# zhuhaozh/metadrive_ped

Hardware: AMD Instinct MI355X
Metric: agent-steps/sec at 4096 envs x 240-beam lidar (higher is better)
Workload: dtype f32; 1 GPU; BASELINE configs[1]: 4096 batched MetaDriveEnv per GPU, 3-block PG map (reference default block distribution: curves, straights, ramps, X/T intersections, roundabouts), 240-beam lidar, traffic_density=0.1, trigger traffic, auto-reset; envs_per_gpu=4096, agents_per_env=1, mover_capacity=24, n_beams=240

## Files before the change

### metadrive_ped_amd/csrc/mdstep.hip

```cpp
#include <hip/hip_runtime.h>
#include <stddef.h>
#include <stdint.h>
#include <stdio.h>
#include <stdlib.h>

#include <type_traits>

#include "md_curriculum.h"
#include "md_expert.h"
#include "md_expert_sense.h"
#include "md_ai_protect.h"
#include "md_scenario.h"
#include "md_topdown.h"
#include "md_render.h"
#include "md_branch.h"
#include "md_ped.h"
#include "md_vector_obs.h"
#include "md_lean_pins.h"
#include "md_lean_view.h"

namespace {

constexpr int kBlock = 256;

enum Phase : int {
    PH_RESET = 1,
    PH_IDM = 2,
    PH_INTEGRATE = 4,
    PH_LOCALIZE = 8,
    PH_CONTACTS = 16,
    PH_TRAFFIC = 32,
    PH_OBSERVE = 64,
    PH_LIDAR = 128,
    PH_LIFECYCLE = 256,
    PH_ALL = 511,
    PH_LOCALIZE_ROAD_FIRST = PH_LOCALIZE | (1 << 20),
};

thread_local char g_err[256] = "ok";

#ifdef MD_STAMP
__device__ unsigned long long* g_stamp_buf = nullptr;
__device__ const int* g_env_order = nullptr;
#define MD_STAMP_AT(i)                                                                         \
    do {                                                                                       \
        if (threadIdx.x == 0 && g_stamp_buf) {                                                 \
            unsigned long long* sb_ = g_stamp_buf + (size_t)blockIdx.x * 32;                   \
            sb_[(i)] = __builtin_readcyclecounter();                                           \
            if ((i) == 0) {                                                                    \
                sb_[12] = __builtin_amdgcn_s_memrealtime();                                    \
                sb_[14] = (unsigned long long)__builtin_amdgcn_s_getreg(63492) |               \
                          ((unsigned long long)__builtin_amdgcn_s_getreg(63508) << 32);        \
            }                                                                                  \
            if ((i) == 11) sb_[13] = __builtin_amdgcn_s_memrealtime();                         \
        }                                                                                      \
    } while (0)
#define MD_FINE_STAMP(cond, i)                                                                 \
    do {                                                                                       \
        if ((cond) && g_stamp_buf) g_stamp_buf[(size_t)blockIdx.x * 32 + 16 + (i)] = __builtin_readcyclecounter(); \
    } while (0)
#define MD_LOC_COUNT(cond, hit)                                                                \
    do {                                                                                       \
        if ((cond) && g_stamp_buf) {                                                           \
            atomicAdd(&g_stamp_buf[(size_t)blockIdx.x * 32 + 16 + 12], 1ull);                  \
            if (hit) atomicAdd(&g_stamp_buf[(size_t)blockIdx.x * 32 + 16 + 13], 1ull);         \
        }                                                                                      \
    } while (0)
#define MD_AHEAD_STAMP(cond, i)                                                                \
    do {                                                                                       \
        if ((cond) && g_stamp_buf) g_stamp_buf[(size_t)blockIdx.x * 32 + (i)] = __builtin_readcyclecounter(); \
    } while (0)
enum : int { MD_AHEAD_EVALUATED = 32, MD_AHEAD_HIT = 40, MD_AHEAD_MISS = 48 };
#define MD_AHEAD_COUNT(cond, what)                                                             \
    do {                                                                                       \
        if ((cond) && g_stamp_buf) atomicAdd(&g_stamp_buf[(size_t)blockIdx.x * 32 + 16 + 12], 1ull << (what)); \
    } while (0)
__device__ unsigned long long* g_contacts_buf = nullptr;
#define MD_CONTACTS_STAMP(cond, i)                                                             \
    do {                                                                                       \
        if ((cond) && g_contacts_buf) g_contacts_buf[(size_t)blockIdx.x * 8 + (i)] = __builtin_readcyclecounter(); \
    } while (0)
#define MD_CONTACTS_COUNT(cond, cells, items)                                                  \
    do {                                                                                       \
        if ((cond) && g_contacts_buf) {                                                        \
            g_contacts_buf[(size_t)blockIdx.x * 8 + 4] += (unsigned long long)(cells);         \
            g_contacts_buf[(size_t)blockIdx.x * 8 + 5] += (unsigned long long)(items);         \
        }                                                                                      \
    } while (0)
#else
#define MD_CONTACTS_STAMP(cond, i) do { } while (0)
#define MD_CONTACTS_COUNT(cond, cells, items) do { } while (0)
#define MD_STAMP_AT(i) do { } while (0)
#define MD_FINE_STAMP(cond, i) do { } while (0)
#define MD_LOC_COUNT(cond, hit) do { } while (0)
#define MD_AHEAD_STAMP(cond, i) do { } while (0)
#define MD_AHEAD_COUNT(cond, what) do { } while (0)
#endif
#ifndef MD_ENV_SKIP
#define MD_ENV_SKIP 0
#endif

__host__ __device__ constexpr uint32_t align_up(uint32_t b, uint32_t a) { return (b + a - 1) & ~(a - 1); }

__device__ __forceinline__ float bcast_f(float v, int src) { return __shfl(v, src, 64); }
__device__ __forceinline__ int bcast_i(int v, int src) { return __shfl(v, src, 64); }

__device__ __forceinline__ void wave_lds_sync() {
    __builtin_amdgcn_fence(__ATOMIC_RELEASE, "wavefront");
    __builtin_amdgcn_wave_barrier();
    __builtin_amdgcn_fence(__ATOMIC_ACQUIRE, "wavefront");
}

#ifndef MD_NT_STAGE
#define MD_NT_STAGE 1
#endif
typedef unsigned int md_u32x4 __attribute__((ext_vector_type(4)));
__device__ __forceinline__ uint4 ld_stream(const uint4* p) {
#if MD_NT_STAGE
    const md_u32x4 v = __builtin_nontemporal_load(reinterpret_cast<const md_u32x4*>(p));
    return make_uint4(v.x, v.y, v.z, v.w);
#else
    return *p;
#endif
}
__device__ __forceinline__ void st_stream(uint4* p, const uint4 v) {
#if MD_NT_STAGE
    md_u32x4 t;
    t.x = v.x; t.y = v.y; t.z = v.z; t.w = v.w;
    __builtin_nontemporal_store(t, reinterpret_cast<md_u32x4*>(p));
#else
    *p = v;
#endif
}
__device__ __forceinline__ void st_stream_f(float* p, float v) {
#if MD_NT_STAGE
    __builtin_nontemporal_store(v, p);
#else
    *p = v;
#endif
}

__device__ __forceinline__ int wave_min_i(int v, bool valid, int none) {
    unsigned long long m = __ballot(valid);
    int best = none;
    while (m) {
        const int l = __ffsll((long long)m) - 1;
        m &= m - 1;
        const int o = __shfl(v, l, 64);
        best = o < best ? o : best;
    }
    return best;
}

template <bool kLdsRow = false>
__device__ __forceinline__ void lidar_item(const MdWorld& w, const MdState& s, const MdConfig& c, int a, int sec, int lane,
                           float* __restrict__ out_row, unsigned long long* det) {
    const MdShape me = s.shape[a];
    const int beam = sec * 64 + lane;
    const bool valid = beam < c.n_beams;
    if (!md_present(me.flags)) {
        if (valid) out_row[beam] = 1.0f;
        return;
    }
    float bc = 1.0f, bs = 0.0f;
    if (valid) {
        bc = w.beam_cs[2 * beam];
        bs = w.beam_cs[2 * beam + 1];
    }
    const float dirx = (bc * me.c - bs * me.s) * c.lidar_range;
    const float diry = (bs * me.c + bc * me.s) * c.lidar_range;

    const int nb = min(64, c.n_beams - sec * 64);
    const float inv_n = __builtin_amdgcn_rcpf((float)c.n_beams);
    const float mid_rev = ((float)(sec * 64) + 0.5f * (float)(nb - 1)) * inv_n;
    const float half_rev = 0.5f * (float)(nb - 1) * inv_n;
    const float ax = __builtin_amdgcn_cosf(mid_rev), ay = __builtin_amdgcn_sinf(mid_rev);
    const float cos_h = __builtin_amdgcn_cosf(half_rev), sin_h = __builtin_amdgcn_sinf(half_rev);
    const float half_span = MD_TWO_PI_F * half_rev;
    const bool narrow = half_span < MD_HALF_PI_F - 0.02f;
    const float wax = ax * me.c - ay * me.s;
    const float way = ay * me.c + ax * me.s;

    float best = 1.0f;
    int best_j = -1;
    for (int j0 = 0; j0 < c.cap; j0 += 64) {
        const int j = j0 + lane;
        MdShape o;
        o.flags = 0;
        if (j < c.cap) o = s.shape[j];
        bool keep = (j < c.cap) && (j != a) && md_present(o.flags);
        if (keep) {
            const float ddx = o.cx - me.cx, ddy = o.cy - me.cy;
            const float d2 = ddx * ddx + ddy * ddy;
            const int k = md_kind_of(o.flags);
            const float rb = (md_is_circle_kind(k) ? o.hl : __builtin_amdgcn_sqrtf(o.hl * o.hl + o.hw * o.hw)) + 0.01f;
            const float reach = c.lidar_range + rb;
            if (d2 > reach * reach * 1.0001f) keep = false;
            else if (d2 > rb * rb) {
                const float inv = __builtin_amdgcn_rsqf(d2);
                const float sin_a = rb * inv;
                const float cos_a = __builtin_amdgcn_sqrtf(md_max(0.0f, 1.0f - sin_a * sin_a));
                if (narrow || half_span + md_asin(md_min(sin_a, 1.0f)) < MD_PI_F - 0.01f) {
                    const float cos_lim = cos_h * cos_a - sin_h * sin_a;
                    const float cos_t = (ddx * wax + ddy * way) * inv;
                    if (cos_t < cos_lim - 2e-3f) keep = false;
                }
            }
        }
        unsigned long long mask = __ballot(keep);
        while (mask) {
            const int k = __ffsll((long long)mask) - 1;
            mask &= mask - 1;
            const float ocx = bcast_f(o.cx, k), ocy = bcast_f(o.cy, k);
            const float oc = bcast_f(o.c, k), os = bcast_f(o.s, k);
            const float ohl = bcast_f(o.hl, k), ohw = bcast_f(o.hw, k);
            const int ofl = bcast_i(o.flags, k);
            const float t = md_ray_shape(me.cx, me.cy, dirx, diry, ocx, ocy, oc, os, ohl, ohw, md_kind_of(ofl));
            if (t < best) {
                best = t;
                best_j = j0 + k;
            }
        }
    }
    if (valid) {
        if (kLdsRow) out_row[beam] = best;
        else st_stream_f(&out_row[beam], best);
    }
    if (det) {
        unsigned long long todo = __ballot(valid && best_j >= 0);
        unsigned long long lo = 0ull, hi = 0ull;
        while (todo) {
            const int k = __ffsll((long long)todo) - 1;
            const int jj = bcast_i(best_j, k);
            todo &= ~__ballot(best_j == jj);
            if (jj < 64) lo |= 1ull << jj;
            else hi |= 1ull << (jj - 64);
        }
        if (lane == 0) {
            if (lo) atomicOr(&det[0], lo);
            if (hi) atomicOr(&det[1], hi);
        }
    }
}

__device__ __forceinline__ void phase_lidar(const MdWorld& w, const MdState& s, const MdConfig& c, int e, int tid, int kWaves,
// ... 340 lines not shown
        else row[out_offset1 + (i - n_beams)] = __int_as_float(l_best[k]);
    }
}

}

#include "parts/localize.inc"
#include "parts/contacts.inc"
#include "parts/idm.inc"
#include "parts/observe.inc"
#include "parts/trigger.inc"
#include "parts/lifecycle.inc"
#include "parts/lean_view.inc"

namespace {

__device__ __forceinline__ void copy16(void* dst, const void* src, int nbytes, int tid, int nthreads) {
    uint4* d = reinterpret_cast<uint4*>(dst);
    const uint4* s = reinterpret_cast<const uint4*>(src);
    for (int i = tid; i < (nbytes >> 4); i += nthreads) d[i] = s[i];
}

constexpr int kStageMaxLanes = 64;
constexpr int kWideMaxEnvs = 640;
constexpr uint32_t kRemovedMark = 0xFFFFFFFFu;

__device__ __forceinline__ int kth_bit(unsigned long long lo, unsigned long long hi, int k) {
    int slot = -1;
    while (k >= 0) {
        if (lo) {
            slot = __ffsll((long long)lo) - 1;
            lo &= lo - 1;
        } else if (hi) {
            slot = 64 + __ffsll((long long)hi) - 1;
            hi &= hi - 1;
        } else {
            return -1;
        }
        --k;
    }
    return slot;
}

struct EnvImage {
    MdShape* shape;
    MdDyn* dyn;
    MdPid* pid;
    MdParam* param;
    MdNav* nav;
    float* action;
    uint32_t* flags;
    int32_t* final_lane;
};

__device__ __forceinline__ MdState local_view(const MdState& gv, const EnvImage& img) {
    MdState s = gv;
    s.shape = img.shape;
    s.dyn = img.dyn;
    s.nav = img.nav;
    s.pid = img.pid;
    s.action = img.action;
    s.flags = img.flags;
    s.param = img.param;
    s.final_lane = img.final_lane;
    return s;
}

struct SlotMask { unsigned long long lo, hi; };
static_assert(MD_MAX_CAP <= 128, "drive_mask: two 64-bit words per env");
__device__ __forceinline__ SlotMask drive_mask(const MdShape* shape, int cap, int lane) {
    SlotMask m = {0ull, 0ull};
    for (int j0 = 0; j0 < cap; j0 += 64) {
        const int j = j0 + lane;
        const unsigned long long mk = __ballot(j < cap && md_drives(shape[j < cap ? j : 0].flags));
        if (j0 == 0) m.lo = mk;
        else m.hi = mk;
    }
    return m;
}
__device__ __forceinline__ SlotMask agent_share(SlotMask m, int agents) {
    m.lo &= agents >= 64 ? ~0ull : ((1ull << agents) - 1ull);
    m.hi &= agents <= 64 ? 0ull : (agents >= 128 ? ~0ull : ((1ull << (agents - 64)) - 1ull));
    return m;
}
__device__ __forceinline__ int popc(SlotMask m) { return __popcll(m.lo) + __popcll(m.hi); }

#ifndef MD_ENV_BLOCK
#define MD_ENV_BLOCK 256
#endif
#ifndef MD_ENV_WAVES_EU
#define MD_ENV_WAVES_EU 7
#endif
__device__ __forceinline__ void lean_pins_fold(MdState& s, MdConfig& c) {
#define MD_PIN_ZERO(f) c.f = 0;
#define MD_PIN_NUL(p) s.p = nullptr;
    MD_LEAN_PINS(MD_PIN_ZERO, MD_PIN_NUL)
#undef MD_PIN_ZERO
#undef MD_PIN_NUL
}
__device__ __forceinline__ void lean_size_pins_fold(MdConfig& c, MdConfig& c_scan) {
#define MD_PIN_EQUALS(f, v) c.f = (v);
#define MD_PIN_AT_MOST(f, v)
    MD_LEAN_SIZE_PINS(MD_PIN_EQUALS, MD_PIN_AT_MOST)
#undef MD_PIN_EQUALS
#undef MD_PIN_AT_MOST
    c_scan = c;
#define MD_PIN_EQUALS(f, v)
#define MD_PIN_AT_MOST(f, v) c_scan.f = min(c.f, (v));
    MD_LEAN_SIZE_PINS(MD_PIN_EQUALS, MD_PIN_AT_MOST)
#undef MD_PIN_EQUALS
#undef MD_PIN_AT_MOST
}

template <int PH, bool RESPAWN, bool MULTI>
constexpr int env_waves_per_eu() { return (PH == PH_ALL && !RESPAWN && !MULTI && MD_ENV_BLOCK >= 128) ? MD_ENV_WAVES_EU : 0; }

struct EnvLds { uint32_t shape, dyn, nav, pid, action, flags, lanes, roads, scratch, param, final_lane, det, onlane, cfl, tk, bytes; };
__host__ __device__ inline EnvLds env_lds(int cap, int agents, int n_lanes, int n_roads, int waves, bool multi, bool lidar_only) {
    EnvLds L;
    L.shape = 0;
    L.dyn = L.shape + (uint32_t)cap * sizeof(MdShape);
    L.nav = L.dyn + (uint32_t)cap * sizeof(MdDyn);
    L.pid = L.nav + (uint32_t)cap * sizeof(MdNav);
    L.action = L.pid + (uint32_t)cap * sizeof(MdPid);
    L.flags = L.action + (uint32_t)cap * 2 * sizeof(float);
    L.lanes = align_up(L.flags + (uint32_t)cap * sizeof(uint32_t), 16);
    L.roads = L.lanes + (uint32_t)n_lanes * sizeof(MdLane);
    L.scratch = L.roads + (uint32_t)n_roads * sizeof(MdRoad);
    L.param = L.scratch + (uint32_t)waves * (multi ? kObsScratch : 48) * sizeof(float);
    L.final_lane = L.param + (uint32_t)cap * sizeof(MdParam);
    L.det = L.final_lane + align_up(cap, 2) * sizeof(int32_t);
    L.onlane = L.det + (uint32_t)agents * 2 * sizeof(unsigned long long);
    L.cfl = L.onlane + (uint32_t)cap * sizeof(uint32_t);
    const uint32_t shared_words = 2 * cap > 8 ? 2 * cap : 8;
    L.tk = L.onlane + shared_words * sizeof(uint32_t);
    L.bytes = lidar_only ? L.dyn : L.tk + 3 * sizeof(int);
    return L;
}

template <int PH, bool STAGE_MAP, bool RESPAWN = false, bool MULTI = false, int BLK = MD_ENV_BLOCK, bool NARROW = false>
__global__ __launch_bounds__(BLK)
__attribute__((amdgpu_waves_per_eu(env_waves_per_eu<PH, RESPAWN, MULTI>() ? env_waves_per_eu<PH, RESPAWN, MULTI>() : 1,
                                   env_waves_per_eu<PH, RESPAWN, MULTI>() ? env_waves_per_eu<PH, RESPAWN, MULTI>() : 8)))
void env_kernel(MdWorld w, MdState g, MdConfig c, float* lidar_out,
                                                  int lidar_stride, int lidar_offset) {
    constexpr int kBlock = BLK;
    constexpr int kWaves = kBlock / 64;
    constexpr bool kIdmKeys = !STAGE_MAP && !RESPAWN && !MULTI;
    constexpr bool kLocRoadFirst = PH == PH_ALL ? kIdmKeys : PH == PH_LOCALIZE_ROAD_FIRST;
    constexpr bool kObsLockstep = MD_OBS_LOCKSTEP && PH == PH_ALL && kIdmKeys;
    constexpr bool kObsAhead = MD_OBS_AHEAD && kObsLockstep && kWaves > 1;
    constexpr bool kContactsFlat = MD_CONTACTS_FLAT && PH == PH_ALL && kIdmKeys;
    constexpr bool kLeanView = MD_LEAN_VIEW && PH == PH_ALL && kIdmKeys && BLK >= 256;
    LeanStageIn lean_in;
    if constexpr (kLeanView) {
        lean_in = lean_stage_in_args(lean_args_entry());
        w = MdWorld{};
        g = MdState{};
        c = MdConfig{};
        c.n_envs = lean_in.n_envs;
        c.cap = lean_in.cap;
        c.agents_per_env = lean_in.agents;
    }
    if constexpr (PH == PH_ALL && !RESPAWN && !MULTI && !STAGE_MAP) lean_pins_fold(g, c);
    static_assert(!NARROW || (PH == PH_ALL && !RESPAWN && !MULTI && !STAGE_MAP), "NARROW: a form of the lean non-staged kernel only");
    MdConfig c_scan = c;
    if constexpr (NARROW) lean_size_pins_fold(c, c_scan);
    if ((int)blockIdx.x >= c.n_envs) return;
#ifdef MD_STAMP
    const int e = g_env_order ? g_env_order[blockIdx.x] : (int)blockIdx.x;
#else
    const int e = blockIdx.x;
#endif
    const int tid = threadIdx.x;
    const int wave = tid >> 6, lane = tid & 63;
    const int cap = c.cap;

    const int n_stage_lanes = STAGE_MAP ? w.max_lanes : 0, n_stage_roads = STAGE_MAP ? w.max_roads : 0;
    constexpr bool kLidarOnly = (PH == PH_LIDAR);
    const EnvLds L = env_lds(cap, c.agents_per_env, n_stage_lanes, n_stage_roads, kWaves, MULTI, kLidarOnly);
    extern __shared__ __attribute__((aligned(16))) unsigned char smem[];
    MdShape* l_shape = reinterpret_cast<MdShape*>(smem + L.shape);
    MdDyn* l_dyn = reinterpret_cast<MdDyn*>(smem + L.dyn);
    MdNav* l_nav = reinterpret_cast<MdNav*>(smem + L.nav);
    MdPid* l_pid = reinterpret_cast<MdPid*>(smem + L.pid);
    float* l_action = reinterpret_cast<float*>(smem + L.action);
    uint32_t* l_flags = reinterpret_cast<uint32_t*>(smem + L.flags);
    MdLane* l_lanes = reinterpret_cast<MdLane*>(smem + L.lanes);
    MdRoad* l_roads = reinterpret_cast<MdRoad*>(smem + L.roads);
    float* l_scratch = reinterpret_cast<float*>(smem + L.scratch) + wave * (MULTI ? kObsScratch : 48);
    MdParam* l_param = reinterpret_cast<MdParam*>(smem + L.param);
    int32_t* l_final = reinterpret_cast<int32_t*>(smem + L.final_lane);
    unsigned long long* l_det = reinterpret_cast<unsigned long long*>(smem + L.det);
    const EnvImage img = {l_shape, l_dyn, l_pid, l_param, l_nav, l_action, l_flags, l_final};
    uint32_t* l_onlane = reinterpret_cast<uint32_t*>(smem + L.onlane);
    uint32_t* l_cfl = reinterpret_cast<uint32_t*>(smem + L.cfl);
    int* l_tk = reinterpret_cast<int*>(smem + L.tk);
    const bool track_det = (PH == PH_ALL) && (RESPAWN || MULTI) && g.detected != nullptr;

    MdState gv = md_env_view(&g, &c, e);
    const MdLane* lanes;
    const MdRoad* roads;
    if constexpr (kLeanView) lean_view_stage_in(gv, lean_in, e, cap, c.agents_per_env);
    const int reset_flag = (PH & PH_RESET) ? gv.need_reset[0] : 0;

    MD_STAMP_AT(0);
    const bool kFusedAct = (PH == PH_ALL) && gv.agent_action != nullptr;
    if (STAGE_MAP) {
        lanes = l_lanes;
        roads = l_roads;
    } else if constexpr (!kLeanView) {
        lanes = w.lanes + w.lane_off[w.env_map[e]];
        roads = w.roads + w.road_off[w.env_map[e]];
    }
    if (kLidarOnly) {
        copy16(l_shape, gv.shape, cap * (int)sizeof(MdShape), tid, kBlock);
    } else if (kBlock >= 256) {
        const int n32 = cap * 2, n64 = cap * 4;
        const uint4* g_shape = reinterpret_cast<const uint4*>(gv.shape);
        const uint4* g_dyn = reinterpret_cast<const uint4*>(gv.dyn);
        const uint4* g_pid = reinterpret_cast<const uint4*>(gv.pid);
        const uint4* g_param = reinterpret_cast<const uint4*>(gv.param);
        const uint4* g_nav = reinterpret_cast<const uint4*>(gv.nav);
        uint4 r_shape, r_dyn, r_pid, r_param, r_nav0;
        float2 r_act;
        uint32_t r_fl;
        int r_fin;
        const bool p32 = tid < n32, pc = tid < cap;
        if (p32) {
            r_shape = ld_stream(&g_shape[tid]);
            r_dyn = ld_stream(&g_dyn[tid]);
            r_pid = ld_stream(&g_pid[tid]);
            r_param = ld_stream(&g_param[tid]);
        }
        if (tid < n64) r_nav0 = ld_stream(&g_nav[tid]);
        if (pc) {
            r_act = (kFusedAct && tid < c.agents_per_env) ? reinterpret_cast<const float2*>(gv.agent_action)[tid]
                                                          : reinterpret_cast<const float2*>(gv.action)[tid];
            r_fl = gv.flags[tid];
            r_fin = gv.final_lane ? gv.final_lane[tid] : 0;
        }
        if constexpr (kLeanView) {
            lean_view_map(&lanes, &roads, lean_args_entry(), e);
            const LeanArgs kb = lean_args_here();
            const int n_envs = c.n_envs, agents = c.agents_per_env;
            lean_arg_copy(w, kb, offsetof(MdStepArgs, w));
            lean_arg_copy(c, kb, offsetof(MdStepArgs, c));
            c.n_envs = n_envs;
            c.cap = cap;
            c.agents_per_env = agents;
            lean_pins_fold(g, c);
            c_scan = c;
            if constexpr (NARROW) lean_size_pins_fold(c, c_scan);
            lean_view_routes(gv, kb, e, cap);
        }
        if (STAGE_MAP) {
            const int m = w.env_map[e];
            const int lo = w.lane_off[m], ro = w.road_off[m];
            copy16(l_lanes, w.lanes + lo, (w.lane_off[m + 1] - lo) * (int)sizeof(MdLane), tid, kBlock);
            copy16(l_roads, w.roads + ro, (w.road_off[m + 1] - ro) * (int)sizeof(MdRoad), tid, kBlock);
        }
        int tid_st = tid;
        if constexpr (kLeanView) asm("" : "+v"(tid_st));
        if (tid_st < n32) {
            reinterpret_cast<uint4*>(l_shape)[tid] = r_shape;
            reinterpret_cast<uint4*>(l_dyn)[tid] = r_dyn;
            reinterpret_cast<uint4*>(l_pid)[tid] = r_pid;
            reinterpret_cast<uint4*>(l_param)[tid] = r_param;
        }
        if (tid_st < n64) reinterpret_cast<uint4*>(l_nav)[tid] = r_nav0;
        for (int i = tid + kBlock; i < n64; i += kBlock) reinterpret_cast<uint4*>(l_nav)[i] = g_nav[i];
        if (tid_st < cap) {
            reinterpret_cast<float2*>(l_action)[tid] = r_act;
            l_flags[tid] = r_fl;
            l_final[tid] = r_fin;
        }
        if (track_det)
            for (int j = tid; j < 2 * c.agents_per_env; j += kBlock) l_det[j] = 0ull;
    } else {
        copy16(l_shape, gv.shape, cap * (int)sizeof(MdShape), tid, kBlock);
        if (STAGE_MAP) {
            const int m = w.env_map[e];
            const int lo = w.lane_off[m], ro = w.road_off[m];
            copy16(l_lanes, w.lanes + lo, (w.lane_off[m + 1] - lo) * (int)sizeof(MdLane), tid, kBlock);
            copy16(l_roads, w.roads + ro, (w.road_off[m + 1] - ro) * (int)sizeof(MdRoad), tid, kBlock);
        }
        copy16(l_dyn, gv.dyn, cap * (int)sizeof(MdDyn), tid, kBlock);
        copy16(l_nav, gv.nav, cap * (int)sizeof(MdNav), tid, kBlock);
        copy16(l_pid, gv.pid, cap * (int)sizeof(MdPid), tid, kBlock);
        copy16(l_param, gv.param, cap * (int)sizeof(MdParam), tid, kBlock);
        for (int j = tid; j < cap; j += kBlock) {
            const float* src = (kFusedAct && j < c.agents_per_env) ? gv.agent_action : gv.action;
            l_action[2 * j] = src[2 * j];
            l_action[2 * j + 1] = src[2 * j + 1];
            l_flags[j] = gv.flags[j];
            l_final[j] = gv.final_lane ? gv.final_lane[j] : 0;
        }
        if (track_det)
            for (int j = tid; j < 2 * c.agents_per_env; j += kBlock) l_det[j] = 0ull;
    }
    const bool do_reset = reset_flag != 0;
    const int just_reset = do_reset ? 1 : 0;
    if (do_reset && !kLidarOnly) {
        __syncthreads();
        if constexpr (kLeanView) lean_view_reset(gv, e, cap);
        copy16(l_shape, gv.shape0, cap * (int)sizeof(MdShape), tid, kBlock);
// ... 19 lines not shown
            if (tid == 0) {
                gv.env_steps[0] = 0;
                int n0 = 0;
                for (int j = 0; j < c.agents_per_env; ++j) n0 += (gv.shape0[j].flags & MD_F_ALIVE) ? 1 : 0;
                gv.next_agent_id[0] = n0;
            }
        }
    }
    MdState s = local_view(gv, img);
    if (kLidarOnly) {
        s = gv;
        s.shape = l_shape;
    }
    if ((MULTI || PH == PH_ALL) && tid == 0) l_tk[0] = l_tk[1] = l_tk[2] = 0;
    if (kObsAhead && tid == 0) reinterpret_cast<int*>(smem + L.scratch)[kAhMark] = 0;
    __syncthreads();
    MD_STAMP_AT(1);
    constexpr bool kTriggerEarly = MD_TRIGGER_EARLY && PH == PH_ALL && kIdmKeys && kWaves > 1;
    constexpr int kTrigWord = (kWaves - 1) * 48 + 46;
    if (kTriggerEarly && wave == kWaves - 1) {
        int min_order, trig_road;
        trigger_search_wave(s, c_scan, lane, &min_order, &trig_road);
        if (lane == 0) {
            int* l_trig = reinterpret_cast<int*>(smem + L.scratch) + kTrigWord;
            l_trig[0] = min_order;
            l_trig[1] = trig_road;
        }
    }

    if ((PH & PH_LIFECYCLE) && MULTI && !just_reset) {
        lifecycle_block(w, s, c, w.env_map[e], tid, kBlock, reinterpret_cast<int*>(l_onlane));
    }

    constexpr bool kFused = (PH == PH_ALL);
    const bool agent_idm = (kFused && !RESPAWN && !MULTI) ? false : (c.agent_idm == MD_AGENT_IDM);
    const bool lane_change = (RESPAWN || MULTI) && c.agent_idm == MD_AGENT_LANE_CHANGE;
    constexpr bool kPlanAhead = kFused && kWaves > 1 && !MULTI;
    const bool plan_ahead = kPlanAhead && !agent_idm;
    if ((PH & PH_IDM) && !just_reset && !plan_ahead) {
        if (wave == 0) trigger_env(lanes, s, c, lane);
        __syncthreads();
        MD_STAMP_AT(2);
        for (int j = (agent_idm ? 0 : c.agents_per_env) + wave; j < cap; j += kWaves) {
            const int f = s.shape[j].flags;
            if (md_drives(f) && (agent_idm || !(f & MD_F_AGENT))) idm_vehicle_wave<kIdmKeys>(w, lanes, roads, s, c, w.env_map[e], j, lane, reinterpret_cast<int*>(l_scratch));
        }
        __syncthreads();
    }
    MD_STAMP_AT(3);
    if ((PH & PH_INTEGRATE) && !just_reset) {
        for (int j = tid; j < cap; j += kBlock) {
            if (lane_change && j < c.agents_per_env) {
                const int f = s.shape[j].flags;
                if (md_drives(f) && !(f & MD_F_SPAWNED)) md_lane_change_act(lanes, roads, &s, j);
            }
            if (RESPAWN) md_advance_mover(&s, &c, j);
            else md_integrate_mover(&s, &c, j);
        }
        if (!RESPAWN)
            for (int j = tid; j < cap; j += kBlock) md_walk_mover(&s, &c, j);
        __syncthreads();
    }
    MD_STAMP_AT(4);
    unsigned long long drv_lo = 0ull, drv_hi = 0ull;
    if (kFused) {
        const SlotMask drv = drive_mask(s.shape, cap, lane);
        drv_lo = drv.lo;
        drv_hi = NARROW ? 0ull : drv.hi;
        const SlotMask adrv = agent_share(drv, c.agents_per_env);
        const unsigned long long adrv_lo = adrv.lo, adrv_hi = NARROW ? 0ull : adrv.hi;
        const int nd = NARROW ? __popcll(drv_lo) : popc(drv), na = NARROW ? __popcll(adrv_lo) : popc(adrv);
        if (MULTI) {
            const int npair = (nd + 1) >> 1;
            for (int guard = 0; guard < npair + na; ++guard) {
                int item = 0;
                if (lane == 0) item = atomicAdd(&l_tk[0], 1);
                item = __builtin_amdgcn_readfirstlane(item);
                if (item < 0 || item >= npair + na) break;
                if (item < na) contacts_vehicle(w, s, c, e, kth_bit(adrv_lo, adrv_hi, item), lane, l_cfl);
                else localize_pair(w, lanes, roads, s, e, kth_bit(drv_lo, drv_hi, 2 * (item - na)), kth_bit(drv_lo, drv_hi, 2 * (item - na) + 1), lane, l_onlane);
            }
        } else if (nd + na <= kWaves) {
            for (int item = wave; item < nd + na; item += kWaves) {
                if (item < nd) {
                    if (!(MD_ENV_SKIP & 4)) localize_vehicle<kLocRoadFirst>(w, lanes, roads, s, e, kth_bit(drv_lo, drv_hi, item), lane, l_onlane);
                } else if (!(MD_ENV_SKIP & 8)) contacts_vehicle<kContactsFlat>(w, s, c, e, kth_bit(adrv_lo, adrv_hi, item - nd), lane, l_cfl);
            }
            if constexpr (kObsAhead) {
                if (nd + na < kWaves && wave == nd + na && !(MD_ENV_SKIP & 16))
                    observe_ahead_wave(lanes, roads, s, c, lane, reinterpret_cast<float*>(smem + L.scratch));
            }
        } else {
            const int npair = (nd + 1) >> 1;
            for (int item = wave; item < npair + na; item += kWaves) {
                if (item < npair) {
                    if (!(MD_ENV_SKIP & 4)) localize_pair<kLocRoadFirst>(w, lanes, roads, s, e, kth_bit(drv_lo, drv_hi, 2 * item), kth_bit(drv_lo, drv_hi, 2 * item + 1), lane, l_onlane);
                } else if (!(MD_ENV_SKIP & 8))
                    contacts_vehicle<kContactsFlat>(w, s, c, e, kth_bit(adrv_lo, adrv_hi, item - npair), lane, l_cfl);
            }
        }
        __syncthreads();
    } else {
        if (PH & PH_LOCALIZE) {
            for (int j = wave; j < cap; j += kWaves) localize_vehicle<kLocRoadFirst>(w, lanes, roads, s, e, j, lane);
            __syncthreads();
        }
        MD_STAMP_AT(5);
        if (PH & PH_CONTACTS) {
            for (int j = wave; j < cap; j += kWaves) contacts_vehicle(w, s, c, e, j, lane);
            __syncthreads();
        }
    }
    MD_STAMP_AT(6);
    if (PH & PH_TRAFFIC) {
        for (int j = tid; j < cap; j += kBlock) {
            const bool drove = kFused ? ((((j < 64) ? (drv_lo >> j) : (drv_hi >> (j - 64))) & 1ull) != 0ull) : false;
            if (kFused && !drove) continue;
            const int f = s.shape[j].flags;
            if (kFused)
                s.flags[j] = l_onlane[j] | ((f & MD_F_AGENT) ? l_cfl[j] : 0u);
            if (md_drives(f) && !(f & MD_F_AGENT) && !(s.flags[j] & MD_FL_ON_LANE)) {
                s.shape[j].flags = f & ~MD_F_ALIVE;
                if (kFused) l_cfl[j] = kRemovedMark;
            }
        }
        if (plan_ahead && wave == kWaves - 1) {
            if (kTriggerEarly) {
                const int* l_trig = reinterpret_cast<const int*>(smem + L.scratch) + kTrigWord;
                trigger_fire_wave(lanes, s, c_scan, lane, __builtin_amdgcn_readfirstlane(l_trig[0]), __builtin_amdgcn_readfirstlane(l_trig[1]));
            } else trigger_env(lanes, s, c_scan, lane);
        }
        __syncthreads();
        if (RESPAWN) {
            if (tid == 0) md_traffic_respawn_env(&w, lanes, &s, &c, w.env_map[e]);
            __syncthreads();
        }
    }
    MD_STAMP_AT(7);
    if (plan_ahead) {
        if (wave == 0) {
            if constexpr (kLeanView) {
                const LeanArgs ko = lean_args_here();
                MdConfig co;
                lean_arg_copy(co, ko, offsetof(MdStepArgs, c));
                co.n_envs = c.n_envs;
                co.cap = cap;
                co.agents_per_env = c.agents_per_env;
                MdConfig co_scan;
                lean_pins_fold(g, co);
                if constexpr (NARROW) lean_size_pins_fold(co, co_scan);
                MdState so = s;
                lean_view_observe(so, ko, e, co.agents_per_env, co.obs_dim);
                if (!(MD_ENV_SKIP & 16))
                    for (int a = 0; a < co.agents_per_env; ++a) observe_agent_wave1<kObsLockstep, kObsAhead>(lanes, roads, so, co, a, just_reset, lane, l_scratch);
            } else if (!(MD_ENV_SKIP & 16))
                for (int a = 0; a < c.agents_per_env; ++a) observe_agent_wave1<kObsLockstep, kObsAhead>(lanes, roads, s, c, a, just_reset, lane, l_scratch);
        } else if (!(MD_ENV_SKIP & 2)) {
            int rank = 0;
            for (int j0 = 0; j0 < cap; j0 += 64) {
                const int jl = j0 + lane;
                const int fl = (jl < cap) ? s.shape[jl].flags : 0;
                unsigned long long mk = __ballot(jl < cap && md_drives(fl) && !(fl & MD_F_AGENT));
                while (mk) {
                    const int j = j0 + __ffsll((long long)mk) - 1;
                    mk &= mk - 1;
                    if (rank % (kWaves - 1) == wave - 1) idm_vehicle_wave<kIdmKeys>(w, lanes, roads, s, c_scan, w.env_map[e], j, lane, reinterpret_cast<int*>(l_scratch));
                    ++rank;
                }
            }
        }
        MD_STAMP_AT(8);
    } else if (PH & PH_OBSERVE) {
        if (MULTI) {
            const int n_grp = (c.agents_per_env + kObsGroups - 1) / kObsGroups;
            for (int guard = 0; guard < n_grp; ++guard) {
                int gi = 0;
                if (lane == 0) gi = atomicAdd(&l_tk[1], 1);
                gi = __builtin_amdgcn_readfirstlane(gi);
                if (gi < 0 || gi >= n_grp) break;
                observe_agent_wave(lanes, roads, s, c, gi * kObsGroups, just_reset, lane, l_scratch);
            }
        } else {
            for (int a = wave; a < c.agents_per_env; a += kWaves) observe_agent_wave1(lanes, roads, s, c, a, just_reset, lane, l_scratch);
        }
        MD_STAMP_AT(8);
    }
    if ((PH & PH_LIDAR) && !(PH == PH_ALL && (MD_ENV_SKIP & 1))) {
        if constexpr (kLeanView) {
            const LeanArgs kl = lean_args_here();
            lidar_out = LEAN_ARG(kl, lidar_out);
            lidar_stride = LEAN_ARG(kl, lidar_stride);
            lidar_offset = LEAN_ARG(kl, lidar_offset);
        }
        if (c.n_beams > 0) phase_lidar(w, s, c_scan, e, tid, kWaves, lidar_out, lidar_stride, lidar_offset, track_det ? l_det : nullptr, PH == PH_ALL ? &l_tk[2] : nullptr);
    }

    MD_STAMP_AT(9);
    if (!kLidarOnly) {
        __syncthreads();
        MD_STAMP_AT(10);
        constexpr bool respawns = (PH & PH_TRAFFIC) && RESPAWN;
        if constexpr (kLeanView) lean_view_write_back(gv, e, cap);
        if (kFused && !MULTI && !do_reset) {
            const bool replay = c.traffic_mode == 3;
            auto dirty = [&](int j) { return replay || md_moves(l_shape[j].flags) || l_cfl[j] == kRemovedMark; };
            for (int i = tid; i < cap * 2; i += kBlock)
                if (dirty(i >> 1)) {
                    st_stream(&reinterpret_cast<uint4*>(gv.shape)[i], reinterpret_cast<const uint4*>(l_shape)[i]);
                    st_stream(&reinterpret_cast<uint4*>(gv.dyn)[i], reinterpret_cast<const uint4*>(l_dyn)[i]);
                    st_stream(&reinterpret_cast<uint4*>(gv.pid)[i], reinterpret_cast<const uint4*>(l_pid)[i]);
                }
            for (int i = tid; i < cap * 4; i += kBlock)
                if (dirty(i >> 2)) st_stream(&reinterpret_cast<uint4*>(gv.nav)[i], reinterpret_cast<const uint4*>(l_nav)[i]);
            for (int j = tid; j < cap; j += kBlock)
                if (dirty(j)) {
                    reinterpret_cast<float2*>(gv.action)[j] = reinterpret_cast<const float2*>(l_action)[j];
                    gv.flags[j] = l_flags[j];
                    if (RESPAWN) gv.final_lane[j] = l_final[j];
                }
            if (track_det)
                for (int j = tid; j < 2 * c.agents_per_env; j += kBlock) gv.detected[j] = l_det[j];
            MD_STAMP_AT(11);
            return;
        }
        if (PH & (PH_RESET | PH_IDM | PH_INTEGRATE | PH_TRAFFIC | PH_OBSERVE | PH_LIFECYCLE)) copy16(gv.shape, l_shape, cap * (int)sizeof(MdShape), tid, kBlock);
        if (MULTI && (PH & (PH_RESET | PH_LIFECYCLE)) && c.random_agent_model && c.is_multi_agent)
            copy16(gv.param, l_param, cap * (int)sizeof(MdParam), tid, kBlock);
        if ((PH & (PH_RESET | PH_INTEGRATE | PH_LIFECYCLE)) || respawns) copy16(gv.dyn, l_dyn, cap * (int)sizeof(MdDyn), tid, kBlock);
        if ((PH & (PH_RESET | PH_IDM | PH_LOCALIZE | PH_OBSERVE | PH_LIFECYCLE)) || respawns) copy16(gv.nav, l_nav, cap * (int)sizeof(MdNav), tid, kBlock);
        if ((PH & (PH_RESET | PH_IDM | PH_OBSERVE | PH_LIFECYCLE)) || respawns || (lane_change && (PH & PH_INTEGRATE)))
            copy16(gv.pid, l_pid, cap * (int)sizeof(MdPid), tid, kBlock);
        if (((PH & (PH_RESET | PH_LIFECYCLE)) && MULTI) || ((PH & (PH_RESET | PH_TRAFFIC)) && RESPAWN)) {
            for (int j = tid; j < cap; j += kBlock) gv.final_lane[j] = l_final[j];
        }
        for (int j = tid; j < cap; j += kBlock) {
            if ((PH & (PH_RESET | PH_IDM | PH_INTEGRATE | PH_LIFECYCLE)) || respawns) {
                gv.action[2 * j] = l_action[2 * j];
                gv.action[2 * j + 1] = l_action[2 * j + 1];
            }
            if ((PH & (PH_RESET | PH_LOCALIZE | PH_CONTACTS | PH_OBSERVE | PH_LIFECYCLE)) || respawns) gv.flags[j] = l_flags[j];
        }
        if (track_det)
            for (int j = tid; j < 2 * c.agents_per_env; j += kBlock) gv.detected[j] = l_det[j];
        if (do_reset && tid == 0) gv.need_reset[0] = 0;
    }
    MD_STAMP_AT(11);
}

#ifndef MD_WAVE_ENVS
#define MD_WAVE_ENVS 4
#endif
constexpr int kWaveEnvs = MD_WAVE_ENVS;

struct WaveEnvLds { uint32_t shape, dyn, pid, param, nav, action, flags, final_lane, onlane, cfl, scratch, det, bytes; };
__host__ __device__ inline WaveEnvLds wave_env_lds(int cap, int agents) {
    WaveEnvLds L;
    L.shape = 0;
    L.dyn = L.shape + (uint32_t)cap * sizeof(MdShape);
    L.pid = L.dyn + (uint32_t)cap * sizeof(MdDyn);
    L.param = L.pid + (uint32_t)cap * sizeof(MdPid);
    L.nav = L.param + (uint32_t)cap * sizeof(MdParam);
    L.action = L.nav + (uint32_t)cap * sizeof(MdNav);
    L.flags = L.action + (uint32_t)cap * 2 * sizeof(float);
    L.final_lane = L.flags + (uint32_t)cap * sizeof(uint32_t);
    L.onlane = L.final_lane + (uint32_t)cap * sizeof(int32_t);
    L.cfl = L.onlane + (uint32_t)cap * sizeof(uint32_t);
    L.scratch = L.cfl + (uint32_t)cap * sizeof(uint32_t);
    L.det = L.scratch + 48 * sizeof(float);
    L.bytes = align_up(L.det + (uint32_t)agents * 2 * sizeof(unsigned long long), 16);
    return L;
}
static_assert((sizeof(MdShape) + sizeof(MdDyn) + sizeof(MdPid) + sizeof(MdParam) + sizeof(MdNav) + 6 * 4) % 8 == 0 && 48 * 4 % 8 == 0,
              "wave_env_lds: the detected sets need 8-B alignment");

template <bool RESPAWN>
__global__ __launch_bounds__(64 * kWaveEnvs) void wave_step_kernel(MdWorld w, MdState g, MdConfig c, float* lidar_out,
                                                                  int lidar_stride, int lidar_offset) {
    if constexpr (!RESPAWN) lean_pins_fold(g, c);
    const int lane = threadIdx.x & 63;
    const int e = blockIdx.x * (blockDim.x >> 6) + (threadIdx.x >> 6);
    if (e >= c.n_envs) return;
    const int cap = c.cap;
    const int A = c.agents_per_env;

    extern __shared__ __attribute__((aligned(16))) unsigned char smem[];
    const WaveEnvLds L = wave_env_lds(cap, A);
    unsigned char* base = smem + __builtin_amdgcn_readfirstlane(threadIdx.x >> 6) * L.bytes;
    MdShape* l_shape = reinterpret_cast<MdShape*>(base + L.shape);
    MdDyn* l_dyn = reinterpret_cast<MdDyn*>(base + L.dyn);
    MdPid* l_pid = reinterpret_cast<MdPid*>(base + L.pid);
    MdParam* l_param = reinterpret_cast<MdParam*>(base + L.param);
    MdNav* l_nav = reinterpret_cast<MdNav*>(base + L.nav);
    float* l_action = reinterpret_cast<float*>(base + L.action);
    uint32_t* l_flags = reinterpret_cast<uint32_t*>(base + L.flags);
    int32_t* l_final = reinterpret_cast<int32_t*>(base + L.final_lane);
    uint32_t* l_onlane = reinterpret_cast<uint32_t*>(base + L.onlane);
    uint32_t* l_cfl = reinterpret_cast<uint32_t*>(base + L.cfl);
    float* l_scratch = reinterpret_cast<float*>(base + L.scratch);
    unsigned long long* l_det = reinterpret_cast<unsigned long long*>(base + L.det);
    const EnvImage img = {l_shape, l_dyn, l_pid, l_param, l_nav, l_action, l_flags, l_final};
    const bool track_det = RESPAWN && g.detected != nullptr;

    const MdState gv = md_env_view(&g, &c, e);
    const int reset_flag = gv.need_reset[0];
    MD_STAMP_AT(0);
    const int m = w.env_map[e];
    const MdLane* lanes = w.lanes + w.lane_off[m];
    const MdRoad* roads = w.roads + w.road_off[m];
    const bool fused_act = gv.agent_action != nullptr;

    {
        const int n32 = cap * 2, n64 = cap * 4;
        const uint4* g_shape = reinterpret_cast<const uint4*>(gv.shape);
        const uint4* g_dyn = reinterpret_cast<const uint4*>(gv.dyn);
        const uint4* g_pid = reinterpret_cast<const uint4*>(gv.pid);
        const uint4* g_param = reinterpret_cast<const uint4*>(gv.param);
        const uint4* g_nav = reinterpret_cast<const uint4*>(gv.nav);
        uint4 r_shape, r_dyn, r_pid, r_param, r_nav0, r_nav1;
        float2 r_act;
        uint32_t r_fl;
        int r_fin;
        const bool p32 = lane < n32, pc = lane < cap;
        if (p32) {
            r_shape = ld_stream(&g_shape[lane]);
            r_dyn = ld_stream(&g_dyn[lane]);
            r_pid = ld_stream(&g_pid[lane]);
            r_param = ld_stream(&g_param[lane]);
        }
        if (lane < n64) r_nav0 = ld_stream(&g_nav[lane]);
        if (lane + 64 < n64) r_nav1 = ld_stream(&g_nav[lane + 64]);
        if (pc) {
            r_act = (fused_act && lane < A) ? reinterpret_cast<const float2*>(gv.agent_action)[lane]
                                            : reinterpret_cast<const float2*>(gv.action)[lane];
            r_fl = gv.flags[lane];
            r_fin = gv.final_lane ? gv.final_lane[lane] : 0;
        }
        if (p32) {
            reinterpret_cast<uint4*>(l_shape)[lane] = r_shape;
            reinterpret_cast<uint4*>(l_dyn)[lane] = r_dyn;
            reinterpret_cast<uint4*>(l_pid)[lane] = r_pid;
            reinterpret_cast<uint4*>(l_param)[lane] = r_param;
        }
        if (lane < n64) reinterpret_cast<uint4*>(l_nav)[lane] = r_nav0;
        if (lane + 64 < n64) reinterpret_cast<uint4*>(l_nav)[lane + 64] = r_nav1;
        if (pc) {
            reinterpret_cast<float2*>(l_action)[lane] = r_act;
            l_flags[lane] = r_fl;
            l_final[lane] = r_fin;
        }
        for (int i = lane + 64; i < n32; i += 64) {
            reinterpret_cast<uint4*>(l_shape)[i] = g_shape[i];
// ... 1463 lines not shown
```

### metadrive_ped_amd/csrc/parts/lean_view.inc

```

namespace {

#ifndef MD_LEAN_VIEW
#define MD_LEAN_VIEW 1
#endif

typedef const __attribute__((address_space(4))) unsigned char* LeanArgs;

__device__ __forceinline__ LeanArgs lean_args_entry() { return (LeanArgs)__builtin_amdgcn_kernarg_segment_ptr(); }
__device__ __forceinline__ LeanArgs lean_args_here() {
    LeanArgs p = lean_args_entry();
    asm volatile("" : "+s"(p));
    return p;
}
__device__ __forceinline__ int lean_here(int v) {
    v = __builtin_amdgcn_readfirstlane(v);
    asm volatile("" : "+s"(v));
    return v;
}
template <typename T>
__device__ __forceinline__ T lean_arg_at(LeanArgs p, size_t off) {
    static_assert(std::is_scalar<T>::value, "lean_arg_at: one pointer or number; lean_arg_copy for a struct");
    return *reinterpret_cast<const __attribute__((address_space(4))) T*>(p + off);
}
#define LEAN_ARG(p, field) lean_arg_at<decltype(static_cast<MdStepArgs*>(nullptr)->field)>((p), offsetof(MdStepArgs, field))
template <typename T>
__device__ __forceinline__ void lean_arg_copy(T& dst, LeanArgs p, size_t off) {
    __builtin_memcpy(&dst, reinterpret_cast<const __attribute__((address_space(4))) T*>(p + off), sizeof(T));
}


struct LeanStageIn {
    int n_envs, agents, cap;
    MdShape* shape; MdDyn* dyn; MdPid* pid; MdParam* param; MdNav* nav; float* action; const float* agent_action;
    uint32_t* flags; int32_t* final_lane; int32_t* need_reset;
};
__device__ __forceinline__ LeanStageIn lean_stage_in_args(LeanArgs p) {
    LeanStageIn a;
    a.n_envs = LEAN_ARG(p, c.n_envs);
    a.agents = LEAN_ARG(p, c.agents_per_env);
    a.cap = LEAN_ARG(p, c.cap);
    a.shape = LEAN_ARG(p, g.shape);
    a.dyn = LEAN_ARG(p, g.dyn);
    a.pid = LEAN_ARG(p, g.pid);
    a.param = LEAN_ARG(p, g.param);
    a.nav = LEAN_ARG(p, g.nav);
    a.action = LEAN_ARG(p, g.action);
    a.agent_action = LEAN_ARG(p, g.agent_action);
    a.flags = LEAN_ARG(p, g.flags);
    a.final_lane = LEAN_ARG(p, g.final_lane);
    a.need_reset = LEAN_ARG(p, g.need_reset);
    asm("" : "+s"(a.n_envs), "+s"(a.agents), "+s"(a.cap)
           : "s"(a.shape), "s"(a.dyn), "s"(a.pid), "s"(a.param), "s"(a.nav), "s"(a.action), "s"(a.agent_action), "s"(a.flags), "s"(a.final_lane),
             "s"(a.need_reset));
    return a;
}
__device__ __forceinline__ void lean_view_stage_in(MdState& v, const LeanStageIn& a, int e, int cap, int agents) {
    const size_t b = (size_t)e * (size_t)cap;
    v.shape = a.shape + b;
    v.dyn = a.dyn + b;
    v.pid = a.pid + b;
    v.param = a.param + b;
    v.nav = a.nav + b;
    v.action = a.action + 2 * b;
    v.agent_action = a.agent_action ? a.agent_action + (size_t)e * agents * 2 : nullptr;
    v.flags = a.flags + b;
    v.final_lane = a.final_lane ? a.final_lane + b : nullptr;
    v.need_reset = a.need_reset + e;
}
__device__ __forceinline__ void lean_view_map(const MdLane** lanes, const MdRoad** roads, LeanArgs p, int e) {
    const int m = LEAN_ARG(p, w.env_map)[e];
    *lanes = LEAN_ARG(p, w.lanes) + LEAN_ARG(p, w.lane_off)[m];
    *roads = LEAN_ARG(p, w.roads) + LEAN_ARG(p, w.road_off)[m];
}
__device__ __forceinline__ void lean_view_write_back(MdState& v, int e, int cap) {
    const LeanArgs p = lean_args_here();
    e = lean_here(e);
    const size_t b = (size_t)e * (size_t)cap;
    v.shape = LEAN_ARG(p, g.shape) + b;
    v.dyn = LEAN_ARG(p, g.dyn) + b;
    v.pid = LEAN_ARG(p, g.pid) + b;
    v.nav = LEAN_ARG(p, g.nav) + b;
    v.action = LEAN_ARG(p, g.action) + 2 * b;
    v.flags = LEAN_ARG(p, g.flags) + b;
    v.need_reset = LEAN_ARG(p, g.need_reset) + e;
}
__device__ __forceinline__ void lean_view_reset(MdState& v, int e, int cap) {
    const LeanArgs p = lean_args_here();
    e = lean_here(e);
    const size_t b = (size_t)e * (size_t)cap;
    v.shape0 = LEAN_ARG(p, g.shape0) + b;
    v.dyn0 = LEAN_ARG(p, g.dyn0) + b;
    v.nav0 = LEAN_ARG(p, g.nav0) + b;
    v.pid0 = LEAN_ARG(p, g.pid0) + b;
}
__device__ __forceinline__ void lean_view_observe(MdState& v, LeanArgs p, int e, int agents, int obs_dim) {
    e = lean_here(e);
    const size_t a = (size_t)e * (size_t)agents;
    v.obs = LEAN_ARG(p, g.obs) + a * (size_t)obs_dim;
    v.reward = LEAN_ARG(p, g.reward) + a;
    v.cost = LEAN_ARG(p, g.cost) + a;
    v.step_info = LEAN_ARG(p, g.step_info) + a * 8;
    uint8_t* done_out = LEAN_ARG(p, g.done_out);
    v.done_out = done_out ? done_out + 4 * a : nullptr;
    v.need_reset = LEAN_ARG(p, g.need_reset) + e;
}
__device__ __forceinline__ void lean_view_routes(MdState& v, LeanArgs p, int e, int cap) {
    const size_t b = (size_t)e * (size_t)cap;
    v.route_nodes = LEAN_ARG(p, g.route_nodes) + b * MD_ROUTE_LEN;
    v.route_roads = LEAN_ARG(p, g.route_roads) + b * MD_ROUTE_LEN;
    v.idm_rand = LEAN_ARG(p, g.idm_rand) + b * MD_IDM_RAND;
    uint32_t* rng = LEAN_ARG(p, g.rng);
    v.rng = rng ? rng + e : nullptr;
}

}
```

Baseline: 67.18 million agent-steps/s.

## Let each wave write back its own slots and skip final block barrier

Adds per-slot write-back ownership. The agent slot is stored by wave 0 after observation, IDM-driven vehicles are stored by the wave that stepped them, and the remaining dirty slots are stored by the last wave. In the non-reset case the kernel then returns early, skipping the __syncthreads and the shared write-back tail. This is meant to remove the block-wide barrier and the serialized store phase. The cost is extra per-wave LDS syncs, and correctness depends on the ownership partition covering every dirty slot exactly once.

```diff
diff --git a/include/md_write_back_own.h b/include/md_write_back_own.h
--- /dev/null
+++ b/include/md_write_back_own.h
@@ -0,0 +1,16 @@
+#ifndef MD_WRITE_BACK_OWN_H
+#define MD_WRITE_BACK_OWN_H
+
+#include "md_entity.h"
+
+enum { MD_WB_NOBODY = 0, MD_WB_WAVE0 = 1, MD_WB_IDM = 2, MD_WB_REST = 3 };
+
+MD_HD int md_wb_dirty(int flags, int removed) { return md_moves(flags) || removed; }
+
+MD_HD int md_wb_owner(int flags, int is_agent, int removed) {
+    if (!is_agent && md_drives(flags)) return MD_WB_IDM;
+    if (!md_wb_dirty(flags, removed)) return MD_WB_NOBODY;
+    return is_agent ? MD_WB_WAVE0 : MD_WB_REST;
+}
+
+#endif
diff --git a/metadrive_ped_amd/csrc/mdstep.hip b/metadrive_ped_amd/csrc/mdstep.hip
--- a/metadrive_ped_amd/csrc/mdstep.hip
+++ b/metadrive_ped_amd/csrc/mdstep.hip
@@ -18,6 +18,7 @@
 #include "md_vector_obs.h"
 #include "md_lean_pins.h"
 #include "md_lean_view.h"
+#include "md_write_back_own.h"
 
 namespace {
 
@@ -53,6 +54,13 @@
                           ((unsigned long long)__builtin_amdgcn_s_getreg(63508) << 32);        \
             }                                                                                  \
             if ((i) == 11) sb_[13] = __builtin_amdgcn_s_memrealtime();                         \
+        }                                                                                      \
+    } while (0)
+#define MD_STAMP_WAVE_END(cond)                                                                \
+    do {                                                                                       \
+        if ((cond) && g_stamp_buf) {                                                           \
+            atomicMax(&g_stamp_buf[(size_t)blockIdx.x * 32 + 11], (unsigned long long)__builtin_readcyclecounter()); \
+            atomicMax(&g_stamp_buf[(size_t)blockIdx.x * 32 + 13], (unsigned long long)__builtin_amdgcn_s_memrealtime()); \
         }                                                                                      \
     } while (0)
 #define MD_FINE_STAMP(cond, i)                                                                 \
@@ -91,6 +99,7 @@
 #define MD_CONTACTS_STAMP(cond, i) do { } while (0)
 #define MD_CONTACTS_COUNT(cond, cells, items) do { } while (0)
 #define MD_STAMP_AT(i) do { } while (0)
+#define MD_STAMP_WAVE_END(cond) do { } while (0)
 #define MD_FINE_STAMP(cond, i) do { } while (0)
 #define MD_LOC_COUNT(cond, hit) do { } while (0)
 #define MD_AHEAD_STAMP(cond, i) do { } while (0)
@@ -737,6 +746,7 @@
     constexpr bool kObsAhead = MD_OBS_AHEAD && kObsLockstep && kWaves > 1;
     constexpr bool kContactsFlat = MD_CONTACTS_FLAT && PH == PH_ALL && kIdmKeys;
     constexpr bool kLeanView = MD_LEAN_VIEW && PH == PH_ALL && kIdmKeys && BLK >= 256;
+    constexpr bool kWriteBackOwn = MD_WRITE_BACK_OWN && kLeanView && MD_ENV_SKIP == 0;
     LeanStageIn lean_in;
     if constexpr (kLeanView) {
         lean_in = lean_stage_in_args(lean_args_entry());
@@ -1062,7 +1072,15 @@
                 MdState so = s;
                 lean_view_observe(so, ko, e, co.agents_per_env, co.obs_dim);
                 if (!(MD_ENV_SKIP & 16))
-                    for (int a = 0; a < co.agents_per_env; ++a) observe_agent_wave1<kObsLockstep, kObsAhead>(lanes, roads, so, co, a, just_reset, lane, l_scratch);
+                    for (int a = 0; a < co.agents_per_env; ++a) {
+                        observe_agent_wave1<kObsLockstep, kObsAhead>(lanes, roads, so, co, a, just_reset, lane, l_scratch);
+                        if (kWriteBackOwn && !do_reset) {
+                            wave_lds_sync();
+                            const int fa = l_shape[a].flags;
+                            if (md_wb_owner(fa, fa & MD_F_AGENT, l_cfl[a] == kRemovedMark) == MD_WB_WAVE0)
+                                lean_store_slot(l_shape, l_dyn, l_pid, l_nav, l_action, l_flags, e, cap, a, lane);
+                        }
+                    }
             } else if (!(MD_ENV_SKIP & 16))
                 for (int a = 0; a < c.agents_per_env; ++a) observe_agent_wave1<kObsLockstep, kObsAhead>(lanes, roads, s, c, a, just_reset, lane, l_scratch);
         } else if (!(MD_ENV_SKIP & 2)) {
@@ -1071,10 +1089,25 @@
                 const int jl = j0 + lane;
                 const int fl = (jl < cap) ? s.shape[jl].flags : 0;
                 unsigned long long mk = __ballot(jl < cap && md_drives(fl) && !(fl & MD_F_AGENT));
+                if (kWriteBackOwn && !do_reset && wave == kWaves - 1) {
+                    const int own = jl < cap ? md_wb_owner(fl, fl & MD_F_AGENT, l_cfl[jl] == kRemovedMark) : MD_WB_NOBODY;
+                    unsigned long long rest = __ballot(own == MD_WB_REST || (own == MD_WB_WAVE0 && jl >= c.agents_per_env));
+                    while (rest) {
+                        const int j = j0 + __ffsll((long long)rest) - 1;
+                        rest &= rest - 1;
+                        lean_store_slot(l_shape, l_dyn, l_pid, l_nav, l_action, l_flags, e, cap, j, lane);
+                    }
+                }
                 while (mk) {
                     const int j = j0 + __ffsll((long long)mk) - 1;
                     mk &= mk - 1;
-                    if (rank % (kWaves - 1) == wave - 1) idm_vehicle_wave<kIdmKeys>(w, lanes, roads, s, c_scan, w.env_map[e], j, lane, reinterpret_cast<int*>(l_scratch));
+                    if (rank % (kWaves - 1) == wave - 1) {
+                        idm_vehicle_wave<kIdmKeys>(w, lanes, roads, s, c_scan, w.env_map[e], j, lane, reinterpret_cast<int*>(l_scratch));
+                        if (kWriteBackOwn && !do_reset) {
+                            wave_lds_sync();
+                            lean_store_slot(l_shape, l_dyn, l_pid, l_nav, l_action, l_flags, e, cap, j, lane);
+                        }
+                    }
                     ++rank;
                 }
             }
@@ -1107,6 +1140,13 @@
 
     MD_STAMP_AT(9);
     if (!kLidarOnly) {
+        if constexpr (kWriteBackOwn) {
+            if (!do_reset) {
+                MD_STAMP_AT(10);
+                MD_STAMP_WAVE_END(lane == 0);
+                return;
+            }
+        }
         __syncthreads();
         MD_STAMP_AT(10);
         constexpr bool respawns = (PH & PH_TRAFFIC) && RESPAWN;
diff --git a/metadrive_ped_amd/csrc/parts/lean_view.inc b/metadrive_ped_amd/csrc/parts/lean_view.inc
--- a/metadrive_ped_amd/csrc/parts/lean_view.inc
+++ b/metadrive_ped_amd/csrc/parts/lean_view.inc
@@ -85,6 +85,26 @@
     v.flags = LEAN_ARG(p, g.flags) + b;
     v.need_reset = LEAN_ARG(p, g.need_reset) + e;
 }
+#ifndef MD_WRITE_BACK_OWN
+#define MD_WRITE_BACK_OWN 1
+#endif
+static_assert(sizeof(MdShape) == 32 && sizeof(MdDyn) == 32 && sizeof(MdPid) == 32 && sizeof(MdNav) == 64, "lean_store_slot: units per record");
+__device__ __forceinline__ void lean_store_slot(const MdShape* l_shape, const MdDyn* l_dyn, const MdPid* l_pid, const MdNav* l_nav,
+                                                const float* l_action, const uint32_t* l_flags, int e, int cap, int j, int lane_id) {
+    const LeanArgs p = lean_args_here();
+    e = lean_here(e);
+    const size_t n = (size_t)e * (size_t)cap + (size_t)j;
+    if (lane_id < 2) {
+        st_stream(reinterpret_cast<uint4*>(LEAN_ARG(p, g.shape) + n) + lane_id, reinterpret_cast<const uint4*>(l_shape + j)[lane_id]);
+        st_stream(reinterpret_cast<uint4*>(LEAN_ARG(p, g.dyn) + n) + lane_id, reinterpret_cast<const uint4*>(l_dyn + j)[lane_id]);
+        st_stream(reinterpret_cast<uint4*>(LEAN_ARG(p, g.pid) + n) + lane_id, reinterpret_cast<const uint4*>(l_pid + j)[lane_id]);
+    }
+    if (lane_id < 4) st_stream(reinterpret_cast<uint4*>(LEAN_ARG(p, g.nav) + n) + lane_id, reinterpret_cast<const uint4*>(l_nav + j)[lane_id]);
+    if (lane_id == 0) {
+        reinterpret_cast<float2*>(LEAN_ARG(p, g.action))[n] = reinterpret_cast<const float2*>(l_action)[j];
+        LEAN_ARG(p, g.flags)[n] = l_flags[j];
+    }
+}
 __device__ __forceinline__ void lean_view_reset(MdState& v, int e, int cap) {
     const LeanArgs p = lean_args_here();
     e = lean_here(e);
```

Result: faster. 68.03 million agent-steps/s, median of 6 (+1.3%).
